# aleximmer/Laplace

Hardware: AMD Instinct MI355X
Metric: KFAC-GGN fit samples/sec, ResNet-18 (higher is better)
Workload: dtype f32 (fp16x2-split products, fp32 accumulate); 1 GPU; c4: ResNet-18 (CIFAR stem, BN frozen) full-network KFAC exact GGN fit, per-GPU minibatch 128, synthetic N(0,1) 3x32x32, 10 classes, N=50000; per_gpu_batch=128, parallelism=dp1, minibatches_in_flight=2

## Files before the change

### include/laplace_hip.h

```cpp
#ifndef LAPLACE_HIP_H
#define LAPLACE_HIP_H

#include <stddef.h>
#include <stdint.h>

#ifdef __cplusplus
extern "C" {
#endif

#define LK_OK 0
#define LK_EINVAL (-1)
#define LK_EWORKSPACE (-2)
#define LK_ELAUNCH (-3)
#define LK_ENOTCONV (-4)

#define LK_GRAM_UPPER_ONLY 1u
#define LK_GRAM_SLABS_PERSIST 2u

int lk_version(void);
const char* lk_last_error(void);

size_t lk_loss_workspace_bytes(int64_t B);
int lk_softmax_hess_sqrt_f32(const float* f, const int64_t* y, int64_t B, int64_t C, float* S,
                             float* loss_accum, float* ws, void* stream);
// ... 125 lines not shown
int lk_copy_absmax_f32(const float* x, float* y, int64_t n, unsigned* amax, void* stream);

int lk_pack_upper_f32(const float* A, int64_t n, float* packed, void* stream);
int lk_unpack_upper_f32(const float* packed, int64_t n, float* A, void* stream);

int lk_gemm_f32(const float* A, const float* B, const float* E, float* C, int64_t batch, int64_t M, int64_t N, int64_t K,
                int64_t lda, int64_t ldb, int64_t ldc, int64_t lde, int64_t stride_a, int64_t stride_b, int64_t stride_c,
                int trans_a, int trans_b, float alpha, int accumulate, void* stream);
int lk_kron_pow_f32(const float* l1, int64_t n1, const float* l2, int64_t n2, const float* delta, float exponent,
                    int damping, float* lam, void* stream);
int lk_unsplit_transpose_f32(const void* x_h, const void* x_l, const int* sexp, int64_t S, int64_t B, int64_t L, int64_t C,
                             float* out, void* stream);
size_t lk_gram_tn_f16x2_workspace_bytes(int64_t R, int64_t C);
int lk_gram_tn_f16x2(const void* x_h, const void* x_l, const int* sexp, int64_t R, int64_t C, float alpha, float* G,
                     const void* zero16, void* ws, size_t ws_bytes, void* stream);

int lk_diag_ggn_linear_f32(const float* a, const float* g, int64_t B, int64_t Cc, int64_t Di, int64_t Do,
                           float alpha, float* h_w, float* h_b, void* stream);

int lk_jac_linear_f32(const float* a, const float* g, int64_t B, int64_t Cc, int64_t Di, int64_t Do,
                      float* Js, int64_t P, int64_t col0, int64_t bcol0, void* stream);
int lk_jac_conv_f32(const float* x_nchw, const float* g, int64_t B, int64_t Cc, int64_t Cin, int64_t H, int64_t W,
                    int64_t Do, int kh, int kw, int sh, int sw, int ph, int pw, int dh, int dw,
                    float* Js, int64_t P, int64_t col0, int64_t bcol0, void* stream);

int lk_jac_norm_affine_f32(const float* g, const float* xhat, int64_t S, int64_t B, int64_t L, int64_t Ch, int layout,
                           float* Js, int64_t P, int64_t wcol0, int64_t bcol0, void* stream);

int lk_jac_norm_affine_nhwc_f16x2(const void* g_h, const void* g_l, const int* sexp, const float* x, const float* mu,
                                  const float* rstd, int64_t S, int64_t B, int64_t L, int64_t Ch, float* Js, int64_t P,
// ... 157 lines not shown
```

### laplace_amd/_lib.py

```python
from __future__ import annotations

import ctypes
import os
from typing import Optional

import torch

_HERE = os.path.dirname(os.path.abspath(__file__))
LIB_PATH = os.environ.get("LK_LIB") or os.path.join(_HERE, "csrc", "liblaplace_hip.so")

LK_GRAM_UPPER_ONLY = 1
LK_GRAM_SLABS_PERSIST = 2

_c_f32p = ctypes.c_void_p
_i64 = ctypes.c_int64
_int = ctypes.c_int
_f32 = ctypes.c_float
_sz = ctypes.c_size_t
_vp = ctypes.c_void_p
_u32 = ctypes.c_uint

SIGNATURES = {
    "lk_version": (_int, []),
    "lk_last_error": (ctypes.c_char_p, []),
# ... 43 lines not shown
    "lk_conv_nhwc_f16x2_vjp": (_int, [_vp, _vp, _vp, _vp, _i64, _i64, _i64, _i64, _vp, _vp, _vp, _vp, _i64, _i64, _i64, _i64,
                                      _vp, _vp, _vp, _vp, _vp, _vp, _int, _vp, _i64, _vp, _vp, _vp, _vp, _vp,
                                      _vp, _int, _vp]),
    "lk_conv_winp_eligible": (_int, [_i64, _i64, _i64, _i64, _i64, _i64, _int]),
    "lk_conv_nhwc_f16x2_vjp_wc": (_int, [_vp, _vp, _vp, _vp, _i64, _i64, _i64, _i64, _vp, _vp, _vp, _vp, _vp, _vp, _i64, _i64, _i64,
                                         _i64, _vp, _vp, _vp, _vp, _vp, _vp, _int, _vp, _i64, _vp, _vp, _vp, _vp, _vp, _vp, _int,
                                         _vp]),
    "lk_conv_nhwc_f16x2_vjp_strided": (_int, [_vp] * 16 + [_i64] * 9 + [_vp, _vp, _vp, _vp, _vp, _vp, _int, _vp, _i64, _vp, _vp, _vp,
                                               _vp, _vp, _vp, _int, _vp]),
    "lk_vjp_nhwc_split_f16x2": (_int, [_vp, _vp, _vp, _vp, _vp, _vp, _int, _vp, _vp, _vp, _i64, _i64, _i64, _vp, _vp, _vp, _vp]),
    "lk_bn_act_fwd_nhwc_f16x2": (_int, [_vp, _vp, _i64, _vp, _vp, _vp, _vp, _vp, _vp, _vp, _vp, _i64, _int, _i64, _i64, _i64, _vp, _vp,
                                        _vp, _vp, _vp, _vp, _vp, _vp]),
    "lk_unsplit_transpose_f32": (_int, [_vp, _vp, _vp, _i64, _i64, _i64, _i64, _vp, _vp]),
    "lk_gram_tn_f16x2_workspace_bytes": (_sz, [_i64, _i64]),
    "lk_gram_tn_f16x2": (_int, [_vp, _vp, _vp, _i64, _i64, _f32, _vp, _vp, _vp, _sz, _vp]),
    "lk_gemm_f32": (_int, [_vp, _vp, _vp, _vp, _i64, _i64, _i64, _i64, _i64, _i64, _i64, _i64, _i64, _i64, _i64, _int, _int, _f32,
                           _int, _vp]),
    "lk_kron_pow_f32": (_int, [_vp, _i64, _vp, _i64, _vp, _f32, _int, _vp, _vp]),
    "lk_pack_upper_f32": (_int, [_vp, _i64, _vp, _vp]),
    "lk_unpack_upper_f32": (_int, [_vp, _i64, _vp, _vp]),
    "lk_symmetrize_f32": (_int, [_vp, _i64, _vp]),
    "lk_permute_sym_f32": (_int, [_vp, _i64, _i64, _vp, _int, _vp]),
    "lk_finalize_factors_f32": (_int, [_i64, _vp, _vp, _vp, _vp, _vp, _vp, _vp]),
    "lk_diag_ggn_linear_f32": (_int, [_vp, _vp, _i64, _i64, _i64, _i64, _f32, _vp, _vp, _vp]),
    "lk_jac_linear_f32": (_int, [_vp, _vp, _i64, _i64, _i64, _i64, _vp, _i64, _i64, _i64, _vp]),
    "lk_jac_conv_f32": (
        _int,
        [_vp, _vp, _i64, _i64, _i64, _i64, _i64, _i64, _int, _int, _int, _int, _int, _int, _int, _int, _vp, _i64, _i64, _i64, _vp],
    ),
    "lk_jac_gconv_f32": (
# ... 700 lines not shown
    def gram_tn_f16x2(self, x, alpha, out):
        _check(out, "out")
        _one_scale(x, "gram_tn_f16x2")
        C = x.planes.shape[-1]
        R = x.planes[0].numel() // C
        nbytes = int(self.lib.lk_gram_tn_f16x2_workspace_bytes(R, C))
        if nbytes == 0 and R:
            raise LaplaceHipError(f"gram_tn_f16x2: C = {C} not supported (64 or a multiple of 128)")
        ws = self._workspace(nbytes, out.device)
        z = self._zero16(out.device)
        self._rc(self._timed("gram16", float(R) * C * (C + 1), out.device, lambda: self.lib.lk_gram_tn_f16x2(
            _ptr(x.planes[0]), _ptr(x.planes[1]), _ptr(x.sexp), R, C, float(alpha), _ptr(out), _ptr(z), _ptr(ws),
            ws.numel(), self._stream(out.device))), "lk_gram_tn_f16x2")
        return out

    def pack_upper(self, A, packed):
        _check(A, "A"), _check(packed, "packed")
        self._rc(self.lib.lk_pack_upper_f32(_ptr(A), A.shape[0], _ptr(packed), self._stream(A.device)), "lk_pack_upper_f32")

    def unpack_upper(self, packed, A):
        _check(A, "A"), _check(packed, "packed")
        self._rc(self.lib.lk_unpack_upper_f32(_ptr(packed), A.shape[0], _ptr(A), self._stream(A.device)), "lk_unpack_upper_f32")

    def gemm(self, A, B, C, batch, M, N, Kd, lda, ldb, ldc, sa=0, sb=0, sc=0, ta=False, tb=False, E=None, lde=0,
             alpha=1.0, accumulate=False):
        self._rc(self.lib.lk_gemm_f32(_ptr(A), _ptr(B), _ptr(E), _ptr(C), batch, M, N, Kd, lda, ldb, ldc, lde, sa, sb, sc,
                                      1 if ta else 0, 1 if tb else 0, float(alpha), 1 if accumulate else 0,
                                      self._stream(C.device)), "lk_gemm_f32")

    def kron_pow(self, l1, l2, delta, exponent, damping=False):
# ... 1002 lines not shown
```

### laplace_amd/backend.py

```python
from __future__ import annotations

import collections
import math
import threading
import os
from collections.abc import MutableMapping

import torch
import torch.nn.functional as F
from torch import nn

from laplace_amd._lib import SplitTensor, get_kernels, is_channels_last, keep_layout
from laplace_amd.capture import NormTapReused, Tape, norm_servable
from laplace_amd.sweep import SeedBatchedSweep, SweepUnsupported
from laplace_amd.sweep_nhwc import NhwcNormGrad, SplitSweep
from laplace_amd.kron import HipKron
from laplace_amd.refapi import EFInterface, GGNInterface


_OWN_ROTATION = True


def shared_operands(tap, g, B, C, Q1=None, Q2=None, bounds=None, planes: bool = True):
    m = tap.module
# ... 357 lines not shown
    def _positions(tap, a) -> int:
        if tap.kind == "conv2d":
            m = tap.module
            H, W = a.shape[-2:]
            oh = (H + 2 * m.padding[0] - m.dilation[0] * (m.kernel_size[0] - 1) - 1) // m.stride[0] + 1
            ow = (W + 2 * m.padding[1] - m.dilation[1] * (m.kernel_size[1] - 1) - 1) // m.stride[1] + 1
            return oh * ow
        return int(a[0].numel() // a.shape[-1])

    def _factor_shapes(self, tap):
        m = tap.module
        if tap.kind == "linear":
            return m.out_features, m.in_features
        return m.out_channels, m.in_channels * m.kernel_size[0] * m.kernel_size[1]

    def _factor_A(self, tap, N, alpha_a_scale, kfac_approx, A, fused=False):
        K = get_kernels()
        a = tap.a.to(torch.float32)
        m = tap.module
        L = self._positions(tap, a)
        if tap.kind == "linear":
            Di = m.in_features
            if kfac_approx == "expand" or L == 1:
                K.gram_tn(a.reshape(-1, Di).contiguous(), alpha_a_scale / (N * L), A, upper_only=fused)
            else:
                K.gram_tn(a.reshape(a.shape[0], L, Di).mean(1).contiguous(), alpha_a_scale / N, A, upper_only=fused)
            return A
        if kfac_approx == "expand":
            ak = keep_layout(a)
            n = A.shape[0]
            if (fused and getattr(K, "use_gram_conv16", False) and hasattr(K, "im2col_split") and m.kernel_size[0] * m.kernel_size[1] > 1
                    and tuple(m.dilation) == (1, 1) and m.stride[0] == m.stride[1] and m.padding[0] == m.padding[1]
                    and m.groups == 1 and isinstance(m.padding[0], int) and ak.is_cuda == A.is_cuda
                    and (n + 127) // 128 * 128 <= 4096 and ak.shape[0] * L * ((n + 127) // 128 * 128) < (1 << 33)):
                Kp = n if (n == 64 or n % 128 == 0) else (64 if n < 64 else (n + 127) // 128 * 128)
                pm = K.im2col_split(ak, m.kernel_size, m.stride[0], m.padding[0], Kp)
                if Kp == n:
                    K.gram_tn_f16x2(pm, alpha_a_scale / (N * L), A)
                else:
                    Ap = torch.zeros(Kp, Kp, dtype=torch.float32, device=A.device)
                    K.gram_tn_f16x2(pm, alpha_a_scale / (N * L), Ap)
                    A += Ap[:n, :n]
                return A
            K.gram_conv(ak, m.kernel_size, m.stride, m.padding, m.dilation, alpha_a_scale / (N * L), A,
                        upper_only=fused, native=fused)
        else:
            cols = torch.nn.functional.unfold(a, m.kernel_size, dilation=m.dilation, padding=m.padding, stride=m.stride)
            if fused:
                KK = m.kernel_size[0] * m.kernel_size[1]
                cols = cols.reshape(cols.shape[0], m.in_channels, KK, -1).transpose(1, 2).reshape(cols.shape)
            K.gram_tn(cols.mean(2).contiguous(), alpha_a_scale / N, A, upper_only=fused)
        return A
# ... 265 lines not shown
_PROCESS_STREAMS_LOCK = threading.Lock()


def _process_streams(key, make):
    with _PROCESS_STREAMS_LOCK:
        return _process_streams_locked(key, make)


def _process_streams_locked(key, make):
    hit = _PROCESS_STREAMS.get(key)
    if hit is None:
        hit = _PROCESS_STREAMS[key] = make()
    return hit


class KronAccumulator:

    use_pixgram = True
    _defer_bn = True
    _persist_slabs = True
    pix_group = 8
    lag_join = True

    def __init__(self, backend, N: int, kfac_approx: str = "expand", overlap: bool = True):
        twin, dt = backend._twin() if hasattr(backend, "_twin") else (None, torch.float32)
        self._caller, self._out_dtype = (backend, dt) if twin is not None else (None, torch.float32)
        if twin is not None:
            backend = twin
        self.backend, self.N, self.kfac_approx = backend, N, kfac_approx
        self.overlap = overlap
# ... 72 lines not shown
            plan = K.pixpair_plan(H, W, Cin, tap.a.device)
            if plan is not None and plan[0] * Cin * Cin * 4 <= (1 << 30):
                return ("pair", H, W, Cin, plan)
        if H * W <= K.pixgram_max_hw and H * W * Cin <= 16384:
            return ("dense", H, W, Cin)
        return None

    def _accumulate_A(self, idx, tap, F, rt):
        K = get_kernels()
        if self.defer_pix:
            geo = self._pix_geometry(tap)
            if geo is not None and geo[0] == "pair" and tap.a.dtype == torch.float32:
                t = K.nchw_to_nhwc(keep_layout(tap.a))
                self._pix_inputs.setdefault(idx, []).append((geo, rt / (self.N * geo[1] * geo[2]), t, tap.module))
                return
            self.backend._factor_A(tap, self.N, rt, self.kfac_approx, F[1], fused=True)
            return
        acc = self._pix.get(idx)
        if acc is None:
            self.backend._factor_A(tap, self.N, rt, self.kfac_approx, F[1], fused=True)
            return
        geo, buf = acc
        alpha = rt / (self.N * geo[1] * geo[2])
        a = keep_layout(tap.a.to(torch.float32))
        if geo[0] != "pair":
            K.pixgram_accumulate(a, alpha, buf)
        elif self.pix_group <= 1:
            K.pixpair_accumulate(a, alpha, buf, geo[4])
        else:
            self._push_pix_input(idx, geo, alpha, a, nhwc=False)

    direct_stack = True

    def _pix_sink(self, name, shape, device):
        idx = self._tap_index.get(name)
# ... 430 lines not shown
            main = torch.cuda.current_stream(f.device)
            side.wait_stream(main)
            with torch.cuda.stream(side):
                for i, (tap, F) in enumerate(zip(tape.taps, self.factors)):
                    self._accumulate_A(i, tap, F, rt)
            self._a_done = torch.cuda.Event()
            self._a_done.record(side)
        else:
            for i, (tap, F) in enumerate(zip(tape.taps, self.factors)):
                self._accumulate_A(i, tap, F, rt)
        seeds, hs = b._kron_seeds(f, y, self.loss)
        defer = getattr(grad_fn, "streams_taps", False) and self._defer_bn
        if getattr(grad_fn, "streams_taps", False):
            by_name = {tap.name: (tap, F) for tap, F in zip(tape.taps, self.factors)}

            def on_tap(name, g):
                tap, F = by_name[name]
                persist = None if isinstance(g, SplitTensor) else self._g_slabs(tap, g, rt * hs)
                if side is None:
                    b._factor_G(tap, g, rt * hs, self.kfac_approx, F[0], fused=True, persist=persist)
                    return
                ev = torch.cuda.Event()
                ev.record(main)
                side.wait_event(ev)
                with torch.cuda.stream(side):
                    b._factor_G(tap, g, rt * hs, self.kfac_approx, F[0], fused=True, persist=persist)
                (g.planes if isinstance(g, SplitTensor) else g).record_stream(side)
                if isinstance(g, SplitTensor) and torch.is_tensor(g.sexp):
                    g.sexp.record_stream(side)

            grad_fn(seeds, stack=False, on_tap=on_tap, defer_bn_scale=defer)
        else:
            grads = grad_fn(seeds, stack=False)
            for tap, g, F in zip(tape.taps, grads, self.factors):
                b._factor_G(tap, g, rt * hs, self.kfac_approx, F[0], fused=True)
        if defer:
            self._note_grad_scales(tape, grad_fn.grad_scale())
        if side is not None:
            if self.lag_join:
                for tap in tape.taps:
                    if torch.is_tensor(tap.a) and tap.a.is_cuda:
                        tap.a.record_stream(side)
                if self._side_done is not None:
                    self._side_older.append(self._side_done)
                while len(self._side_older) >= self.lag_depth and self._side_older:
                    main.wait_event(self._side_older.pop(0))
# ... 8 lines not shown
            return None
        K = get_kernels()
        S, B, Do = g.shape[0], g.shape[1], g.shape[2]
        L = g.shape[3] * g.shape[4]
        need = K.gram_nt_slab_bytes(S * B, Do, L)
        idx = self._tap_index[tap.name]
        cur = self._gslabs.get(idx)
        if cur is not None and (cur[0].numel() < need or cur[2] != L or cur[3] != alpha):
            self._flush_g_slabs(only=idx)
            cur = None
        if cur is None:
            cur = (torch.zeros(need, dtype=torch.uint8, device=g.device), Do, L, alpha)
            self._gslabs[idx] = cur
        return cur[0]

    def _raw_tensors(self):
        return [t for F in self.factors for t in F] + [self.loss]

    def _raw_compatible(self, other) -> bool:
        return (self.factors is not None and other.factors is not None and not other._pix
                and not other._pix_pending and not self._gslabs and not other._gslabs
                and (not (self._pix or self._pix_pending) or all(g[0] == "pair" for g, _ in self._pix.values()))
                and self.N == other.N and self.kfac_approx == other.kfac_approx and self.backend is other.backend
                and self._taps_meta == other._taps_meta and len(self.factors) == len(other.factors)
                and all(a.shape == b.shape for a, b in zip(self._raw_tensors(), other._raw_tensors()))
                and set(self._gscale) == set(other._gscale)
                and all(self._gscale[k] is other._gscale[k] or torch.equal(self._gscale[k], other._gscale[k])
                        for k in self._gscale))

    def clone(self) -> "KronAccumulator":
        self._fold_lanes()
        self._join_side()
        new = KronAccumulator(self.backend, self.N, self.kfac_approx, self.overlap)
        new._caller, new._out_dtype, new.coalesce = self._caller, self._out_dtype, self.coalesce
        new.use_pixgram, new._persist_slabs = self.use_pixgram, self._persist_slabs
        new.defer_pix, new.pix_group = self.defer_pix, self.pix_group
        new._pix_inputs = {k: list(v) for k, v in self._pix_inputs.items()}
        if self.factors is not None:
            if self._gslabs or any(g[0] != "pair" for g, _ in self._pix.values()):
                raise RuntimeError("clone() of an accumulator with dense pixel-pair / slab state is not supported")
            for idx in list(self._pix_pending):
                self._drain_pixpair(idx)
            new.factors = [[t.clone() for t in F] for F in self.factors]
            new.loss = self.loss.clone()
            new._taps_meta = list(self._taps_meta)
            new._gscale = dict(self._gscale)
            new._tap_index = dict(self._tap_index)
            new._pix = {idx: (geo, buf.clone()) for idx, (geo, buf) in self._pix.items()}
            new._pix_pending, new._gslabs = {}, {}
            new._side = self._side
        return new

    def merge_(self, other: "KronAccumulator") -> bool:
        self._fold_lanes()
        other._fold_lanes()
        if not self._raw_compatible(other):
            return False
        skip = set(other._pix_inputs)
        mine = [t for i, F in enumerate(self.factors) for j, t in enumerate(F) if not (j == 1 and i in skip)] + [self.loss]
        theirs = [t for i, F in enumerate(other.factors) for j, t in enumerate(F) if not (j == 1 and i in skip)] + [other.loss]
        side = self._side or other._side
        if side is None or not self.lag_join or not self.loss.is_cuda:
            self._join_side()
            other._join_side()
            torch._foreach_add_(mine, theirs)
            self._push_adopted(self._adopt_pix_inputs(other))
        else:
            self._side = side
            main = torch.cuda.current_stream(self.loss.device)
            if self._side_done is not None:
# ... 11 lines not shown
            self._side_done = torch.cuda.Event()
            self._side_done.record(side)
        return True

    def _join_side(self):
        if self._side is not None:
            torch.cuda.current_stream(self._side.device).wait_stream(self._side)
            self._side_done = None
            self._side_older = []

    def _flush_g_slabs(self, only=None):
        K = get_kernels()
        if self._gslabs:
            self._join_side()
        for idx in ([only] if only is not None else list(self._gslabs)):
            buf, n, L, alpha = self._gslabs.pop(idx)
            K.gram_slabs_reduce(buf, n, L, alpha, self.factors[idx][0], upper_only=True)

    def _note_grad_scales(self, tape, scales):
        for idx, tap in enumerate(tape.taps):
            s_new = scales.get(tap.name)
            s_old = self._gscale.get(idx)
            if s_old is None:
                if s_new is not None:
                    self._gscale[idx] = s_new
            elif s_new is None or (s_new is not s_old and not torch.equal(s_new, s_old)):
                raise RuntimeError(f"{tap.name}: the BatchNorm scale changed during the fit (model not in eval mode?)")

    def _apply_grad_scales(self):
        self._join_side()
        for idx, s_ in self._gscale.items():
            G = self.factors[idx][0]
            G.mul_(s_.reshape(-1, 1) * s_.reshape(1, -1))
        self._gscale = {}

    def tensors(self) -> list[torch.Tensor]:
        self._fold_lanes()
        self._resolve_pix_inputs()
        self._flush_pixgrams()
        self._flush_g_slabs()
        self._apply_grad_scales()
        out = CurvatureExchange([t for F in self.factors for t in F] + [self.loss])
        out.owner = self
        return out

    def finalize(self):
        K = get_kernels()
        rt = math.sqrt(float(self.backend.factor))
# ... 212 lines not shown
```

### laplace_amd/csrc/lk_sweep16.hip

```cpp
#include "lk_common.h"
#include "lk_split16.h"

namespace lk {

typedef short s16x4 __attribute__((ext_vector_type(4)));

template <bool MFLOAT>
__global__ __launch_bounds__(256) void vjp_nhwc_split_kernel(
    const float* __restrict__ g, const unsigned* __restrict__ g_amax, const _Float16* __restrict__ g2h,
    const _Float16* __restrict__ g2l, const int* __restrict__ g2_sexp, const void* __restrict__ m,
    const unsigned* __restrict__ m_amax, const float* __restrict__ scale, const unsigned* __restrict__ scale_amax, int C,
    int S, int64_t per8, _Float16* __restrict__ oh, _Float16* __restrict__ ol, int* __restrict__ out_sexp) {
  float bound = 0.f;
  if (g) bound += __uint_as_float(g_amax[0]);
  const VjpScale vs = vjp_bound_scale<true>(bound, g2h != nullptr, g2_sexp, m != nullptr, MFLOAT, m_amax, scale != nullptr, scale_amax);
  const float sc_out = exp2i_sat(vs.so);
  if (blockIdx.x == 0 && threadIdx.x == 0) out_sexp[0] = vs.so;
  const int64_t e8 = (int64_t)blockIdx.x * 256 + threadIdx.x;
  if (e8 >= per8) return;
  float mult[8];
#pragma unroll
  for (int j = 0; j < 8; ++j) mult[j] = sc_out;
  if (m) {
    if (MFLOAT) vjp_mult8_times(mult, reinterpret_cast<const float*>(m) + 8 * e8);
// ... 136 lines not shown
__device__ __forceinline__ float gram16_unscale_add(float old, float v, float alpha, float inv) {
  return __builtin_fmaf(alpha, (v * inv) * inv, old);
}

typedef __attribute__((address_space(3))) void lds_void16;
typedef __attribute__((address_space(1))) const void gbl_void16;

struct Gram16Tnp {
  const int* tiles;
  int ldc;
  const int* sexp;
  float alpha;
  float* blocks;
};

template <int NB, int BKR, int KW, bool TNP>
__global__ __launch_bounds__(256) void gram16_kernel(const _Float16* __restrict__ Xh, const _Float16* __restrict__ Xl,
                                                     int64_t R, int64_t C, int64_t rows_per_split,
                                                     const _Float16* __restrict__ zero16, float* __restrict__ ws,
                                                     int nbc, const Gram16Tnp tp) {
  using G = Gram16Cfg<NB, BKR, KW>;
  constexpr int TW = G::TW;
  extern __shared__ __attribute__((aligned(16))) char smem[];
  const int tid = threadIdx.x, lane = tid & 63, wave = tid >> 6;
  int bi = 0, bj = 0;
  int64_t colA = 0, colB = 0, out_off = 0;
  if constexpr (TNP) {
    const int nblk = gridDim.x;
    int bid = blockIdx.x;
    bid = xcd_tile_order(bid, nblk);
    colA = tp.tiles[3 * bid], colB = tp.tiles[3 * bid + 1], out_off = tp.tiles[3 * bid + 2];
  } else {
    int p = blockIdx.x;
    while (p >= nbc - bi) p -= nbc - bi, ++bi;
    bj = bi + p;
    colA = (int64_t)bi * NB, colB = (int64_t)bj * NB;
  }
// ... 45 lines not shown

  auto load_frag = [&](const char* plane, int k16, int col0) -> f16x8 {
    s16x4 v[2];
#pragma unroll
    for (int j = 0; j < 2; ++j) {
      const int row = k16 * 16 + f_row + j * 4;
      const int col = col0 + f_col;
      const int off = row * G::PITCH + (((col >> 5) ^ gram16_swz<NB>(row)) << 6) + (col & 31) * 2;
      const unsigned addr = (unsigned)(uintptr_t)(__attribute__((address_space(3))) const char*)(plane + off);
      asm volatile("ds_read_b64_tr_b16 %0, %1" : "=v"(v[j]) : "v"(addr));
    }
    const f16x4 f0 = __builtin_bit_cast(f16x4, v[0]), f1 = __builtin_bit_cast(f16x4, v[1]);
    return f16x8{f0[0], f0[1], f0[2], f0[3], f1[0], f1[1], f1[2], f1[3]};
  };

  constexpr int NOLD = TNP ? (KW == 4 ? TW * TW * 4 : TW * TW * 16) : 1;
  float old[NOLD];
  if constexpr (TNP) {
    const int lr_ = lane & 31, lh_ = lane >> 5;
    if (KW == 4) {
#pragma unroll
      for (int i = 0; i < NOLD; ++i) {
        const int e = tid + 256 * i, t = e >> 10, a = t / TW, b = t % TW, row = (e >> 5) & 31, col = e & 31;
        old[i] = tp.blocks[out_off + (int64_t)(a * 32 + row) * tp.ldc + b * 32 + col];
      }
    } else {
#pragma unroll
      for (int a = 0; a < TW; ++a)
#pragma unroll
        for (int b = 0; b < TW; ++b)
#pragma unroll
          for (int r = 0; r < 16; ++r) {
// ... 33 lines not shown
#pragma unroll
      for (int a = 0; a < TW; ++a)
#pragma unroll
        for (int b = 0; b < TW; ++b) {
          if (diag && wr == wc && a > b) continue;
          f32x16 c = acc[a][b];
          c = __builtin_amdgcn_mfma_f32_32x32x16_f16(al[a], bh[b], c, 0, 0, 0);
          c = __builtin_amdgcn_mfma_f32_32x32x16_f16(ah[a], bl[b], c, 0, 0, 0);
          c = __builtin_amdgcn_mfma_f32_32x32x16_f16(ah[a], bh[b], c, 0, 0, 0);
          acc[a][b] = c;
        }
    }
  }

  const int lr = lane & 31, lh = lane >> 5;
  float* blk = TNP ? nullptr : ws + ((int64_t)blockIdx.y * gridDim.x + blockIdx.x) * (NB * NB);
  if (KW == 4) {
    __syncthreads();
    float* red = reinterpret_cast<float*>(smem);
#pragma unroll
    for (int a = 0; a < TW; ++a)
#pragma unroll
      for (int b = 0; b < TW; ++b) {
        if (!TNP && a > b) continue;
#pragma unroll
        for (int r = 0; r < 16; ++r) {
          const int row = (r & 3) + 8 * (r >> 2) + 4 * lh;
          red[((wave * TW + a) * TW + b) * 1024 + row * 32 + lr] = acc[a][b][r];
        }
      }
    __syncthreads();
    float inv = 0.f;
    if constexpr (TNP) inv = exp2i_sat(-tp.sexp[0]);
#pragma unroll
    for (int i = 0; i < TW * TW * 4; ++i) {
      const int e = tid + 256 * i;
      const int t = e >> 10, a = t / TW, b = t % TW;
      if (!TNP && a > b) continue;
      const float v = ((red[e] + red[TW * TW * 1024 + e]) + red[2 * TW * TW * 1024 + e]) + red[3 * TW * TW * 1024 + e];
      const int row = (e >> 5) & 31, col = e & 31;
      if constexpr (TNP) tp.blocks[out_off + (int64_t)(a * 32 + row) * tp.ldc + b * 32 + col] = gram16_unscale_add(old[i], v, tp.alpha, inv);
      else blk[(a * 32 + row) * NB + b * 32 + col] = v;
    }
    return;
  }
  if (!wave_active) return;
  float inv = 0.f;
  if constexpr (TNP) inv = exp2i_sat(-tp.sexp[0]);
#pragma unroll
  for (int a = 0; a < TW; ++a)
#pragma unroll
    for (int b = 0; b < TW; ++b) {
      if (diag && wr == wc && a > b) continue;
#pragma unroll
      for (int r = 0; r < 16; ++r) {
        const int row = wr * 64 + a * 32 + (r & 3) + 8 * (r >> 2) + 4 * lh;
        const int col = wc * 64 + b * 32 + lr;
        if constexpr (TNP)
          tp.blocks[out_off + (int64_t)row * tp.ldc + col] = gram16_unscale_add(old[(a * TW + b) * 16 + r], acc[a][b][r], tp.alpha, inv);
        else blk[row * NB + col] = acc[a][b][r];
      }
    }
}

template <int NB>
__global__ __launch_bounds__(256) void gram16_reduce4_kernel(const float* __restrict__ ws, int nparts, int npairs, int nbc,
                                                             int C, const int* __restrict__ sexp, float alpha,
                                                             float* __restrict__ Gm) {
  __shared__ float4 red[4][64];
  const int pair = blockIdx.y;
  int bi = 0, bj = 0;
  {
    int p = pair;
    while (p >= nbc - bi) p -= nbc - bi, ++bi;
// ... 91 lines not shown
             "lk_unsplit_transpose_f32: bad arguments (S * B <= 65535)");
  LK_REQUIRE(L <= 65535 * 32ll, "lk_unsplit_transpose_f32: L too large for grid.y (L <= %lld positions)", 65535 * 32ll);
  LK_REQUIRE(C < (1ll << 31) - 32, "lk_unsplit_transpose_f32: C too large (C < 2^31 - 32 channels)");
  if (S * B == 0 || L == 0 || C == 0) return LK_OK;
  hipLaunchKernelGGL(unsplit_transpose_kernel, dim3((unsigned)((C + 31) / 32), (unsigned)((L + 31) / 32), (unsigned)(S * B)),
                     dim3(256), 0, (hipStream_t)stream, (const _Float16*)x_h, (const _Float16*)x_l, sexp, (int)S, (int)B,
                     (int)L, (int)C, out);
  return check_launch("unsplit_transpose_kernel");
}

namespace {
struct Gram16Plan {
  int nb, nbc, npairs, kw, bkr;
  int64_t nsplit, rows_per_split, nparts;
};
Gram16Plan gram16_plan(int64_t R, int64_t C) {
  Gram16Plan p;
  p.nb = C == 64 ? 64 : 128;
  p.kw = C == 64 ? 4 : 1;
  p.bkr = C == 64 ? 64 : 32;
  p.nbc = (int)(C / p.nb);
  p.npairs = p.nbc * (p.nbc + 1) / 2;
  int64_t want = (512 + p.npairs - 1) / p.npairs;
  int64_t stages = (R + p.bkr - 1) / p.bkr;
  int64_t per = (stages + want - 1) / want;
  if (per < 8) per = 8;
  p.rows_per_split = per * p.bkr;
  p.nsplit = (R + p.rows_per_split - 1) / p.rows_per_split;
  if (p.nsplit < 1) p.nsplit = 1;
  p.nparts = p.nsplit;
  return p;
}
}

extern "C" size_t lk_gram_tn_f16x2_workspace_bytes(int64_t R, int64_t C) {
  if (C < 64 || (C != 64 && C % 128)) return 0;
  const Gram16Plan p = gram16_plan(R, C);
  return (size_t)p.nparts * p.npairs * p.nb * p.nb * sizeof(float);
}

extern "C" int lk_gram_tn_f16x2(const void* x_h, const void* x_l, const int* sexp, int64_t R, int64_t C, float alpha,
                                float* Gm, const void* zero16, void* ws, size_t ws_bytes, void* stream) {
  LK_REQUIRE(x_h && x_l && sexp && Gm && zero16 && ws && R >= 0, "lk_gram_tn_f16x2: null pointer");
  LK_REQUIRE(C == 64 || (C >= 128 && C % 128 == 0 && C <= 4096), "lk_gram_tn_f16x2: C must be 64 or a multiple of 128");
  if (R == 0) return LK_OK;
  const Gram16Plan p = gram16_plan(R, C);
  LK_REQUIRE(ws_bytes >= lk_gram_tn_f16x2_workspace_bytes(R, C), "lk_gram_tn_f16x2: workspace too small");
  hipStream_t st = (hipStream_t)stream;
  dim3 grid((unsigned)p.npairs, (unsigned)p.nsplit);
  if (C == 64) {
    using Gc = Gram16Cfg<64, 64, 4>;
    hipLaunchKernelGGL((gram16_kernel<64, 64, 4, false>), grid, dim3(256), 2 * Gc::STAGE, st, (const _Float16*)x_h,
                       (const _Float16*)x_l, R, C, p.rows_per_split, (const _Float16*)zero16, (float*)ws, p.nbc, Gram16Tnp{});
  } else {
    using Gc = Gram16Cfg<128, 32, 1>;
    hipLaunchKernelGGL((gram16_kernel<128, 32, 1, false>), grid, dim3(256), 2 * Gc::STAGE, st, (const _Float16*)x_h,
                       (const _Float16*)x_l, R, C, p.rows_per_split, (const _Float16*)zero16, (float*)ws, p.nbc, Gram16Tnp{});
  }
  int rc = check_launch("gram16_kernel");
  if (rc != LK_OK) return rc;
  dim3 rgrid((unsigned)(p.nb * p.nb / 256), (unsigned)p.npairs);
  if (C == 64)
    hipLaunchKernelGGL(gram16_reduce4_kernel<64>, rgrid, dim3(256), 0, st, (const float*)ws, (int)p.nparts, p.npairs, p.nbc,
                       (int)C, sexp, alpha, Gm);
  else
    hipLaunchKernelGGL(gram16_reduce4_kernel<128>, rgrid, dim3(256), 0, st, (const float*)ws, (int)p.nparts, p.npairs, p.nbc,
                       (int)C, sexp, alpha, Gm);
  return check_launch("gram16_reduce4_kernel");
}

namespace lk {
struct Pix13Args {
  const _Float16 *xh, *xl;
  const _Float16* zero16;
  const int* slots;
  const int* sexp;
  float* blocks;
  float alpha;
  int R, H, W;
};

__device__ __forceinline__ f16x8 pix13_frag(unsigned plane, int lane, int col0) {
  const int grp = lane >> 4, r16 = lane & 15;
// ... 145 lines not shown
extern "C" int lk_conv3x3_pixpair_accumulate_f16x2(const void* x_h, const void* x_l, const int* sexp, int64_t B, int64_t H,
                                                   int64_t W, int64_t Cin, float alpha, float* blocks,
                                                   const int32_t* tiles_dev, int64_t n_tiles, const void* zero16,
                                                   void* stream) {
  LK_REQUIRE(x_h && x_l && sexp && blocks && tiles_dev && zero16 && B >= 0 && n_tiles >= 0,
             "lk_conv3x3_pixpair_accumulate_f16x2: bad arguments");
  LK_REQUIRE(Cin >= 64 && Cin % 64 == 0 && n_tiles < (1ll << 31) && H * W * Cin < (1ll << 31),
             "lk_conv3x3_pixpair_accumulate_f16x2: needs Cin % 64 == 0");
  if (B == 0 || n_tiles == 0) return LK_OK;
  Gram16Tnp tp;
  tp.tiles = tiles_dev, tp.ldc = (int)Cin, tp.sexp = sexp, tp.alpha = alpha, tp.blocks = blocks;
  hipStream_t st = (hipStream_t)stream;
  const int64_t ld = H * W * Cin;
  if (Cin % 128) {
    using Gc = Gram16Cfg<64, 64, 4>;
    hipLaunchKernelGGL((gram16_kernel<64, 64, 4, true>), dim3((unsigned)n_tiles), dim3(256), 2 * Gc::STAGE, st,
                       (const _Float16*)x_h, (const _Float16*)x_l, B, ld, B, (const _Float16*)zero16, (float*)nullptr, 0, tp);
  } else {
    using Gc = Gram16Cfg<128, 32, 1>;
    hipLaunchKernelGGL((gram16_kernel<128, 32, 1, true>), dim3((unsigned)n_tiles), dim3(256), 2 * Gc::STAGE, st,
                       (const _Float16*)x_h, (const _Float16*)x_l, B, ld, B, (const _Float16*)zero16, (float*)nullptr, 0, tp);
  }
  return check_launch("gram16_kernel<pixel pairs>");
}
```

Baseline: 21190 samples/s.

## Accumulate f16x2 Gram factors into persistent slabs and batch same-shape layers per launch

Adds a persistent-slab mode for the fp16x2 Gram kernel: each minibatch's contribution is read-modify-written into per-layer slab buffers, and the cross-split reduction into the Kronecker factor is deferred to flush time instead of running every minibatch. Gradient taps of identical shape are grouped (up to 8) into a single launch using a z-dimension layer table, and the split plan accounts for the layer count. This is meant to cut per-minibatch reduce kernels and launch overhead, at the cost of extra slab memory and a read of the old slab values in every accumulate.

Measured after the change: 21290 samples/s (median of 6 runs). Within noise of the previous version (+0.5%).

```diff
diff --git a/include/laplace_hip.h b/include/laplace_hip.h
--- a/include/laplace_hip.h
+++ b/include/laplace_hip.h
@@ -163,6 +163,13 @@
 size_t lk_gram_tn_f16x2_workspace_bytes(int64_t R, int64_t C);
 int lk_gram_tn_f16x2(const void* x_h, const void* x_l, const int* sexp, int64_t R, int64_t C, float alpha, float* G,
                      const void* zero16, void* ws, size_t ws_bytes, void* stream);
+int lk_gram16_plan(int64_t R, int64_t C, int layers, int64_t* out);
+size_t lk_gram16_slab_bytes(int64_t R, int64_t C, int layers);
+int lk_gram16_accumulate(const void* const* x_h, const void* const* x_l, const int* const* sexp, const float* alpha,
+                         float* const* slabs, int layers, int64_t R, int64_t C, size_t slab_bytes, const void* zero16,
+                         void* stream);
+int lk_gram16_slabs_reduce(const float* slabs, size_t slab_bytes, int64_t R, int64_t C, int layers, float* G,
+                           const void* zero16, void* stream);
 
 int lk_diag_ggn_linear_f32(const float* a, const float* g, int64_t B, int64_t Cc, int64_t Di, int64_t Do,
                            float alpha, float* h_w, float* h_b, void* stream);
diff --git a/laplace_amd/_lib.py b/laplace_amd/_lib.py
--- a/laplace_amd/_lib.py
+++ b/laplace_amd/_lib.py
@@ -81,6 +81,10 @@
     "lk_unsplit_transpose_f32": (_int, [_vp, _vp, _vp, _i64, _i64, _i64, _i64, _vp, _vp]),
     "lk_gram_tn_f16x2_workspace_bytes": (_sz, [_i64, _i64]),
     "lk_gram_tn_f16x2": (_int, [_vp, _vp, _vp, _i64, _i64, _f32, _vp, _vp, _vp, _sz, _vp]),
+    "lk_gram16_plan": (_int, [_i64, _i64, _int, _vp]),
+    "lk_gram16_slab_bytes": (_sz, [_i64, _i64, _int]),
+    "lk_gram16_accumulate": (_int, [_vp, _vp, _vp, _vp, _vp, _int, _i64, _i64, _sz, _vp, _vp]),
+    "lk_gram16_slabs_reduce": (_int, [_vp, _sz, _i64, _i64, _int, _vp, _vp, _vp]),
     "lk_gemm_f32": (_int, [_vp, _vp, _vp, _vp, _i64, _i64, _i64, _i64, _i64, _i64, _i64, _i64, _i64, _i64, _i64, _int, _int, _f32,
                            _int, _vp]),
     "lk_kron_pow_f32": (_int, [_vp, _i64, _vp, _i64, _vp, _f32, _int, _vp, _vp]),
@@ -811,6 +815,50 @@
             ws.numel(), self._stream(out.device))), "lk_gram_tn_f16x2")
         return out
 
+    use_gram16_persist = True
+    gram16_group = True
+    GRAM16_MAX_LAYERS = 8
+
+    def gram16_plan(self, R, C, layers=1):
+        o = (ctypes.c_int64 * 4)()
+        if self.lib.lk_gram16_plan(int(R), int(C), int(layers), o) != 0:
+            return None
+        return dict(nb=o[0], npairs=o[1], nsplit=o[2], rows_per_split=o[3])
+
+    def gram16_slab_bytes(self, R, C, layers=1) -> int:
+        return int(self.lib.lk_gram16_slab_bytes(int(R), int(C), int(layers)))
+
+    def gram16_accumulate(self, xs, alphas, slabs):
+        n = len(xs)
+        if not 1 <= n <= self.GRAM16_MAX_LAYERS or len(alphas) != n or len(slabs) != n:
+            raise LaplaceHipError(f"gram16_accumulate: 1 to {self.GRAM16_MAX_LAYERS} layers, one alpha and one slab buffer each")
+        C = xs[0].planes.shape[-1]
+        R = xs[0].planes[0].numel() // C
+        for x, s in zip(xs, slabs):
+            _one_scale(x, "gram16_accumulate")
+            _check(s, "slabs")
+            if x.planes.shape[-1] != C or x.planes[0].numel() != R * C:
+                raise LaplaceHipError("gram16_accumulate: the layers of one launch share [rows, C]")
+        nbytes = self.gram16_slab_bytes(R, C, n)
+        if nbytes == 0 and R:
+            raise LaplaceHipError(f"gram16_accumulate: C = {C} not supported (64 or a multiple of 128)")
+        if min(s.numel() for s in slabs) * 4 < nbytes:
+            raise LaplaceHipError("gram16_accumulate: persistent slab buffer too small")
+        dev = slabs[0].device
+        arr = lambda ts: (ctypes.c_void_p * n)(*[t.data_ptr() for t in ts])
+        xh, xl, se, sl = arr([x.planes[0] for x in xs]), arr([x.planes[1] for x in xs]), arr([x.sexp for x in xs]), arr(slabs)
+        al = (ctypes.c_float * n)(*[float(a) for a in alphas])
+        z = self._zero16(dev)
+        self._rc(self._timed("gram16", float(n) * R * C * (C + 1), dev, lambda: self.lib.lk_gram16_accumulate(
+            xh, xl, se, al, sl, n, R, C, nbytes, _ptr(z), self._stream(dev))), "lk_gram16_accumulate")
+
+    def gram16_slabs_reduce(self, slabs, R, C, layers, out):
+        _check(out, "out"), _check(slabs, "slabs")
+        self._rc(self.lib.lk_gram16_slabs_reduce(_ptr(slabs), slabs.numel() * 4, int(R), int(C), int(layers), _ptr(out),
+                                                 _ptr(self._zero16(out.device)), self._stream(out.device)),
+                 "lk_gram16_slabs_reduce")
+        return out
+
     def pack_upper(self, A, packed):
         _check(A, "A"), _check(packed, "packed")
         self._rc(self.lib.lk_pack_upper_f32(_ptr(A), A.shape[0], _ptr(packed), self._stream(A.device)), "lk_pack_upper_f32")
diff --git a/laplace_amd/backend.py b/laplace_amd/backend.py
--- a/laplace_amd/backend.py
+++ b/laplace_amd/backend.py
@@ -395,7 +395,7 @@
             return m.out_features, m.in_features
         return m.out_channels, m.in_channels * m.kernel_size[0] * m.kernel_size[1]
 
-    def _factor_A(self, tap, N, alpha_a_scale, kfac_approx, A, fused=False):
+    def _factor_A(self, tap, N, alpha_a_scale, kfac_approx, A, fused=False, slabs16=None):
         K = get_kernels()
         a = tap.a.to(torch.float32)
         m = tap.module
@@ -416,7 +416,9 @@
                     and (n + 127) // 128 * 128 <= 4096 and ak.shape[0] * L * ((n + 127) // 128 * 128) < (1 << 33)):
                 Kp = n if (n == 64 or n % 128 == 0) else (64 if n < 64 else (n + 127) // 128 * 128)
                 pm = K.im2col_split(ak, m.kernel_size, m.stride[0], m.padding[0], Kp)
-                if Kp == n:
+                if slabs16 is not None:
+                    K.gram16_accumulate([pm], [alpha_a_scale / (N * L)], [slabs16(pm, Kp, n)])
+                elif Kp == n:
                     K.gram_tn_f16x2(pm, alpha_a_scale / (N * L), A)
                 else:
                     Ap = torch.zeros(Kp, Kp, dtype=torch.float32, device=A.device)
@@ -712,6 +714,29 @@
     return hit
 
 
+class Gram16Groups:
+
+    def __init__(self, group_max):
+        self.group_max = max(int(group_max), 1)
+        self.held = []
+
+    def _take(self):
+        group, self.held = self.held, []
+        return group
+
+    def add(self, idx, g):
+        out = []
+        if self.held and (tuple(self.held[0][1].shape) != tuple(g.shape) or any(i == idx for i, _ in self.held)):
+            out.append(self._take())
+        self.held.append((idx, g))
+        if g.shape[-1] < 128 or len(self.held) >= self.group_max:
+            out.append(self._take())
+        return out
+
+    def end(self):
+        return [self._take()] if self.held else []
+
+
 class KronAccumulator:
 
     use_pixgram = True
@@ -814,11 +839,11 @@
                 t = K.nchw_to_nhwc(keep_layout(tap.a))
                 self._pix_inputs.setdefault(idx, []).append((geo, rt / (self.N * geo[1] * geo[2]), t, tap.module))
                 return
-            self.backend._factor_A(tap, self.N, rt, self.kfac_approx, F[1], fused=True)
+            self.backend._factor_A(tap, self.N, rt, self.kfac_approx, F[1], fused=True, slabs16=self._a16_slabs(idx))
             return
         acc = self._pix.get(idx)
         if acc is None:
-            self.backend._factor_A(tap, self.N, rt, self.kfac_approx, F[1], fused=True)
+            self.backend._factor_A(tap, self.N, rt, self.kfac_approx, F[1], fused=True, slabs16=self._a16_slabs(idx))
             return
         geo, buf = acc
         alpha = rt / (self.N * geo[1] * geo[2])
@@ -1279,8 +1304,37 @@
         if getattr(grad_fn, "streams_taps", False):
             by_name = {tap.name: (tap, F) for tap, F in zip(tape.taps, self.factors)}
 
+            K16 = get_kernels()
+            persist16 = bool(getattr(K16, "use_gram16_persist", False)) and self._persist_slabs and self.kfac_approx == "expand"
+            group_max = int(getattr(K16, "GRAM16_MAX_LAYERS", 1)) if persist16 and getattr(K16, "gram16_group", False) else 1
+            groups = Gram16Groups(group_max)
+
+            def launch(group):
+                idxs, gs = [i for i, _ in group], [g for _, g in group]
+                C = gs[0].shape[-1]
+                R = gs[0].planes[0].numel() // C
+                slabs = [self._g16_slabs(("g16", i), R, C, len(gs), gs[0].planes.device) for i in idxs]
+                if side is None:
+                    K16.gram16_accumulate(gs, [rt * hs] * len(gs), slabs)
+                    return
+                ev = torch.cuda.Event()
+                ev.record(main)
+                side.wait_event(ev)
+                with torch.cuda.stream(side):
+                    K16.gram16_accumulate(gs, [rt * hs] * len(gs), slabs)
+                for g in gs:
+                    g.planes.record_stream(side)
+                    g.sexp.record_stream(side)
+
             def on_tap(name, g):
                 tap, F = by_name[name]
+                if persist16 and isinstance(g, SplitTensor) and torch.is_tensor(g.sexp) and g.sexp.numel() == 1 \
+                        and (g.shape[-1] == 64 or g.shape[-1] % 128 == 0) and g.shape[-1] <= 4096:
+                    for group in groups.add(self._tap_index[name], g):
+                        launch(group)
+                    return
+                for group in groups.end():
+                    launch(group)
                 persist = None if isinstance(g, SplitTensor) else self._g_slabs(tap, g, rt * hs)
                 if side is None:
                     b._factor_G(tap, g, rt * hs, self.kfac_approx, F[0], fused=True, persist=persist)
@@ -1294,7 +1348,12 @@
                 if isinstance(g, SplitTensor) and torch.is_tensor(g.sexp):
                     g.sexp.record_stream(side)
 
-            grad_fn(seeds, stack=False, on_tap=on_tap, defer_bn_scale=defer)
+            try:
+                grad_fn(seeds, stack=False, on_tap=on_tap, defer_bn_scale=defer)
+                for group in groups.end():
+                    launch(group)
+            finally:
+                groups.held = []
         else:
             grads = grad_fn(seeds, stack=False)
             for tap, g, F in zip(tape.taps, grads, self.factors):
@@ -1333,6 +1392,22 @@
             self._gslabs[idx] = cur
         return cur[0]
 
+    def _g16_slabs(self, key, R, C, layers, device, n=None):
+        cur = self._gslabs.get(key)
+        if cur is not None and cur[1:4] != (R, C, layers):
+            self._flush_g_slabs(only=key)
+            cur = None
+        if cur is None:
+            nbytes = get_kernels().gram16_slab_bytes(R, C, layers)
+            cur = (torch.zeros(nbytes // 4, dtype=torch.float32, device=device), R, C, layers, n)
+            self._gslabs[key] = cur
+        return cur[0]
+
+    def _a16_slabs(self, idx):
+        if not (self._persist_slabs and getattr(get_kernels(), "use_gram16_persist", False)):
+            return None
+        return lambda pm, Kp, n: self._g16_slabs(("a16", idx), pm.planes[0].numel() // Kp, Kp, 1, pm.planes.device, n)
+
     def _raw_tensors(self):
         return [t for F in self.factors for t in F] + [self.loss]
 
@@ -1356,6 +1431,7 @@
         new.defer_pix, new.pix_group = self.defer_pix, self.pix_group
         new._pix_inputs = {k: list(v) for k, v in self._pix_inputs.items()}
         if self.factors is not None:
+            self._flush_g_slabs()
             if self._gslabs or any(g[0] != "pair" for g, _ in self._pix.values()):
                 raise RuntimeError("clone() of an accumulator with dense pixel-pair / slab state is not supported")
             for idx in list(self._pix_pending):
@@ -1373,6 +1449,9 @@
     def merge_(self, other: "KronAccumulator") -> bool:
         self._fold_lanes()
         other._fold_lanes()
+        for acc in (self, other):
+            if acc.factors is not None:
+                acc._flush_g_slabs()
         if not self._raw_compatible(other):
             return False
         skip = set(other._pix_inputs)
@@ -1414,6 +1493,18 @@
         if self._gslabs:
             self._join_side()
         for idx in ([only] if only is not None else list(self._gslabs)):
+            if isinstance(idx, tuple):
+                buf, R, C, layers, n = self._gslabs.pop(idx)
+                F = self.factors[idx[1]][0 if idx[0] == "g16" else 1]
+                if n is None or n == C:
+                    K.gram16_slabs_reduce(buf, R, C, layers, F)
+                else:
+                    Fp = torch.zeros(C, C, dtype=torch.float32, device=F.device)
+                    K.gram16_slabs_reduce(buf, R, C, layers, Fp)
+                    F += Fp[:n, :n]
+                if buf.is_cuda:
+                    buf.record_stream(torch.cuda.current_stream(buf.device))
+                continue
             buf, n, L, alpha = self._gslabs.pop(idx)
             K.gram_slabs_reduce(buf, n, L, alpha, self.factors[idx][0], upper_only=True)
 
@@ -1432,6 +1523,8 @@
         for idx, s_ in self._gscale.items():
             G = self.factors[idx][0]
             G.mul_(s_.reshape(-1, 1) * s_.reshape(1, -1))
+        if self._gscale:
+            self._defer_bn = False
         self._gscale = {}
 
     def tensors(self) -> list[torch.Tensor]:
diff --git a/laplace_amd/csrc/lk_sweep16.hip b/laplace_amd/csrc/lk_sweep16.hip
--- a/laplace_amd/csrc/lk_sweep16.hip
+++ b/laplace_amd/csrc/lk_sweep16.hip
@@ -174,13 +174,32 @@
   float* blocks;
 };
 
-template <int NB, int BKR, int KW, bool TNP>
+constexpr int GRAM16_MAX_LAYERS = 8;
+struct Gram16Layer {
+  const _Float16 *xh, *xl;
+  const int* sexp;
+  float* slabs;
+  float alpha;
+};
+struct Gram16Batch {
+  Gram16Layer l[GRAM16_MAX_LAYERS];
+};
+
+template <int NB, int BKR, int KW, bool ACC, bool TNP>
 __global__ __launch_bounds__(256) void gram16_kernel(const _Float16* __restrict__ Xh, const _Float16* __restrict__ Xl,
                                                      int64_t R, int64_t C, int64_t rows_per_split,
                                                      const _Float16* __restrict__ zero16, float* __restrict__ ws,
-                                                     int nbc, const Gram16Tnp tp) {
+                                                     int nbc, const Gram16Tnp tp, const Gram16Batch bt) {
   using G = Gram16Cfg<NB, BKR, KW>;
   constexpr int TW = G::TW;
+  static_assert(!(ACC && TNP), "the pixel-pair form owns its blocks already");
+  constexpr bool RMW = ACC || TNP;
+  float acc_alpha = 0.f;
+  const int* acc_sexp = nullptr;
+  if constexpr (ACC) {
+    const Gram16Layer& ly = bt.l[blockIdx.z];
+    Xh = ly.xh, Xl = ly.xl, ws = ly.slabs, acc_alpha = ly.alpha, acc_sexp = ly.sexp;
+  }
   extern __shared__ __attribute__((aligned(16))) char smem[];
   const int tid = threadIdx.x, lane = tid & 63, wave = tid >> 6;
   int bi = 0, bj = 0;
@@ -256,8 +275,30 @@
     return f16x8{f0[0], f0[1], f0[2], f0[3], f1[0], f1[1], f1[2], f1[3]};
   };
 
-  constexpr int NOLD = TNP ? (KW == 4 ? TW * TW * 4 : TW * TW * 16) : 1;
+  constexpr int NOLD = RMW ? (KW == 4 ? TW * TW * 4 : TW * TW * 16) : 1;
   float old[NOLD];
+  [[maybe_unused]] float* const acc_blk = ACC ? ws + ((int64_t)blockIdx.y * gridDim.x + blockIdx.x) * (NB * NB) : nullptr;
+  if constexpr (ACC) {
+    const int lr_ = lane & 31, lh_ = lane >> 5;
+    if (KW == 4) {
+#pragma unroll
+      for (int i = 0; i < NOLD; ++i) {
+        const int e = tid + 256 * i, t = e >> 10, a = t / TW, b = t % TW, row = (e >> 5) & 31, col = e & 31;
+        old[i] = a > b ? 0.f : acc_blk[(a * 32 + row) * NB + b * 32 + col];
+      }
+    } else if (wave_active) {
+#pragma unroll
+      for (int a = 0; a < TW; ++a)
+#pragma unroll
+        for (int b = 0; b < TW; ++b)
+#pragma unroll
+          for (int r = 0; r < 16; ++r) {
+            const int row = wr * 64 + a * 32 + (r & 3) + 8 * (r >> 2) + 4 * lh_;
+            const int col = wc * 64 + b * 32 + lr_;
+            old[(a * TW + b) * 16 + r] = (diag && wr == wc && a > b) ? 0.f : acc_blk[row * NB + col];
+          }
+    }
+  }
   if constexpr (TNP) {
     const int lr_ = lane & 31, lh_ = lane >> 5;
     if (KW == 4) {
@@ -321,7 +362,7 @@
   }
 
   const int lr = lane & 31, lh = lane >> 5;
-  float* blk = TNP ? nullptr : ws + ((int64_t)blockIdx.y * gridDim.x + blockIdx.x) * (NB * NB);
+  float* blk = RMW ? nullptr : ws + ((int64_t)blockIdx.y * gridDim.x + blockIdx.x) * (NB * NB);
   if (KW == 4) {
     __syncthreads();
     float* red = reinterpret_cast<float*>(smem);
@@ -339,6 +380,7 @@
     __syncthreads();
     float inv = 0.f;
     if constexpr (TNP) inv = exp2i_sat(-tp.sexp[0]);
+    if constexpr (ACC) inv = exp2i_sat(-acc_sexp[0]);
 #pragma unroll
     for (int i = 0; i < TW * TW * 4; ++i) {
       const int e = tid + 256 * i;
@@ -347,6 +389,7 @@
       const float v = ((red[e] + red[TW * TW * 1024 + e]) + red[2 * TW * TW * 1024 + e]) + red[3 * TW * TW * 1024 + e];
       const int row = (e >> 5) & 31, col = e & 31;
       if constexpr (TNP) tp.blocks[out_off + (int64_t)(a * 32 + row) * tp.ldc + b * 32 + col] = gram16_unscale_add(old[i], v, tp.alpha, inv);
+      else if constexpr (ACC) acc_blk[(a * 32 + row) * NB + b * 32 + col] = gram16_unscale_add(old[i], v, acc_alpha, inv);
       else blk[(a * 32 + row) * NB + b * 32 + col] = v;
     }
     return;
@@ -354,6 +397,7 @@
   if (!wave_active) return;
   float inv = 0.f;
   if constexpr (TNP) inv = exp2i_sat(-tp.sexp[0]);
+  if constexpr (ACC) inv = exp2i_sat(-acc_sexp[0]);
 #pragma unroll
   for (int a = 0; a < TW; ++a)
 #pragma unroll
@@ -365,6 +409,8 @@
         const int col = wc * 64 + b * 32 + lr;
         if constexpr (TNP)
           tp.blocks[out_off + (int64_t)row * tp.ldc + col] = gram16_unscale_add(old[(a * TW + b) * 16 + r], acc[a][b][r], tp.alpha, inv);
+        else if constexpr (ACC)
+          acc_blk[row * NB + col] = gram16_unscale_add(old[(a * TW + b) * 16 + r], acc[a][b][r], acc_alpha, inv);
         else blk[row * NB + col] = acc[a][b][r];
       }
     }
@@ -486,14 +532,15 @@
   int nb, nbc, npairs, kw, bkr;
   int64_t nsplit, rows_per_split, nparts;
 };
-Gram16Plan gram16_plan(int64_t R, int64_t C) {
+Gram16Plan gram16_plan(int64_t R, int64_t C, int layers = 1) {
   Gram16Plan p;
   p.nb = C == 64 ? 64 : 128;
   p.kw = C == 64 ? 4 : 1;
   p.bkr = C == 64 ? 64 : 32;
   p.nbc = (int)(C / p.nb);
   p.npairs = p.nbc * (p.nbc + 1) / 2;
-  int64_t want = (512 + p.npairs - 1) / p.npairs;
+  const int64_t tiles = (int64_t)p.npairs * layers;
+  int64_t want = (512 + tiles - 1) / tiles;
   int64_t stages = (R + p.bkr - 1) / p.bkr;
   int64_t per = (stages + want - 1) / want;
   if (per < 8) per = 8;
@@ -522,12 +569,12 @@
   dim3 grid((unsigned)p.npairs, (unsigned)p.nsplit);
   if (C == 64) {
     using Gc = Gram16Cfg<64, 64, 4>;
-    hipLaunchKernelGGL((gram16_kernel<64, 64, 4, false>), grid, dim3(256), 2 * Gc::STAGE, st, (const _Float16*)x_h,
-                       (const _Float16*)x_l, R, C, p.rows_per_split, (const _Float16*)zero16, (float*)ws, p.nbc, Gram16Tnp{});
+    hipLaunchKernelGGL((gram16_kernel<64, 64, 4, false, false>), grid, dim3(256), 2 * Gc::STAGE, st, (const _Float16*)x_h,
+                       (const _Float16*)x_l, R, C, p.rows_per_split, (const _Float16*)zero16, (float*)ws, p.nbc, Gram16Tnp{}, Gram16Batch{});
   } else {
     using Gc = Gram16Cfg<128, 32, 1>;
-    hipLaunchKernelGGL((gram16_kernel<128, 32, 1, false>), grid, dim3(256), 2 * Gc::STAGE, st, (const _Float16*)x_h,
-                       (const _Float16*)x_l, R, C, p.rows_per_split, (const _Float16*)zero16, (float*)ws, p.nbc, Gram16Tnp{});
+    hipLaunchKernelGGL((gram16_kernel<128, 32, 1, false, false>), grid, dim3(256), 2 * Gc::STAGE, st, (const _Float16*)x_h,
+                       (const _Float16*)x_l, R, C, p.rows_per_split, (const _Float16*)zero16, (float*)ws, p.nbc, Gram16Tnp{}, Gram16Batch{});
   }
   int rc = check_launch("gram16_kernel");
   if (rc != LK_OK) return rc;
@@ -539,6 +586,109 @@
     hipLaunchKernelGGL(gram16_reduce4_kernel<128>, rgrid, dim3(256), 0, st, (const float*)ws, (int)p.nparts, p.npairs, p.nbc,
                        (int)C, sexp, alpha, Gm);
   return check_launch("gram16_reduce4_kernel");
+}
+
+static int gram16_check_shape(const char* fn, int64_t R, int64_t C, int layers) {
+  LK_REQUIRE(layers >= 1 && layers <= GRAM16_MAX_LAYERS, "%s: layers out of range (1 <= layers <= %d)", fn, GRAM16_MAX_LAYERS);
+  LK_REQUIRE(C == 64 || (C >= 128 && C % 128 == 0 && C <= 4096), "%s: C must be 64 or a multiple of 128 (<= 4096)", fn);
+  LK_REQUIRE(R >= 0 && R < (1ll << 40) / C, "%s: extent out of range (0 <= R, R * C < 2^40)", fn);
+  return LK_OK;
+}
+
+static bool gram16_shape_ok(int64_t R, int64_t C, int layers) {
+  return layers >= 1 && layers <= GRAM16_MAX_LAYERS && (C == 64 || (C >= 128 && C % 128 == 0 && C <= 4096)) && R >= 0 &&
+         R < (1ll << 40) / C;
+}
+
+static int gram16_check_plan(int64_t R, int64_t C, int layers, const int64_t* out) {
+  LK_REQUIRE(out, "lk_gram16_plan: null pointer");
+  return gram16_check_shape("lk_gram16_plan", R, C, layers);
+}
+
+static size_t gram16_slab_bytes(int64_t R, int64_t C, int layers) {
+  const Gram16Plan p = gram16_plan(R, C, layers);
+  return (size_t)p.nsplit * p.npairs * p.nb * p.nb * sizeof(float);
+}
+
+static int gram16_check_accumulate(const void* const* x_h, const void* const* x_l, const int* const* sexp, const float* alpha,
+                                   float* const* slabs, int layers, int64_t R, int64_t C, size_t slab_bytes,
+                                   const void* zero16) {
+  const char* fn = "lk_gram16_accumulate";
+  LK_REQUIRE(x_h && x_l && sexp && alpha && slabs && zero16, "%s: null pointer", fn);
+  int rc = gram16_check_shape(fn, R, C, layers);
+  if (rc != LK_OK) return rc;
+  for (int i = 0; i < layers; ++i)
+    LK_REQUIRE(x_h[i] && x_l[i] && sexp[i] && slabs[i], "%s: null pointer in the table entry of layer %d", fn, i);
+  for (int i = 0; i < layers; ++i)
+    for (int j = i + 1; j < layers; ++j)
+      LK_REQUIRE(slabs[i] != slabs[j], "%s: layers %d and %d share their slabs (a tile has one writer per launch)", fn, i, j);
+  LK_REQUIRE(slab_bytes >= gram16_slab_bytes(R, C, layers), "%s: slabs too small (lk_gram16_slab_bytes, each layer's own)", fn);
+  return LK_OK;
+}
+
+static int gram16_check_reduce(const float* slabs, size_t slab_bytes, int64_t R, int64_t C, int layers, const float* Gm,
+                               const void* zero16) {
+  const char* fn = "lk_gram16_slabs_reduce";
+  LK_REQUIRE(slabs && Gm && zero16, "%s: null pointer", fn);
+  int rc = gram16_check_shape(fn, R, C, layers);
+  if (rc != LK_OK) return rc;
+  LK_REQUIRE(slab_bytes >= gram16_slab_bytes(R, C, layers), "%s: slabs too small (lk_gram16_slab_bytes)", fn);
+  return LK_OK;
+}
+
+extern "C" int lk_gram16_plan(int64_t R, int64_t C, int layers, int64_t* out) {
+  int rc = gram16_check_plan(R, C, layers, out);
+  if (rc != LK_OK) return rc;
+  const Gram16Plan p = gram16_plan(R, C, layers);
+  out[0] = p.nb, out[1] = p.npairs, out[2] = p.nsplit, out[3] = p.rows_per_split;
+  return LK_OK;
+}
+
+extern "C" size_t lk_gram16_slab_bytes(int64_t R, int64_t C, int layers) {
+  return gram16_shape_ok(R, C, layers) ? gram16_slab_bytes(R, C, layers) : 0;
+}
+
+extern "C" int lk_gram16_accumulate(const void* const* x_h, const void* const* x_l, const int* const* sexp,
+                                    const float* alpha, float* const* slabs, int layers, int64_t R, int64_t C,
+                                    size_t slab_bytes, const void* zero16, void* stream) {
+  int rc = gram16_check_accumulate(x_h, x_l, sexp, alpha, slabs, layers, R, C, slab_bytes, zero16);
+  if (rc != LK_OK || R == 0) return rc;
+  Gram16Batch bt{};
+  for (int i = 0; i < layers; ++i) {
+    bt.l[i].xh = (const _Float16*)x_h[i], bt.l[i].xl = (const _Float16*)x_l[i], bt.l[i].sexp = sexp[i];
+    bt.l[i].slabs = slabs[i], bt.l[i].alpha = alpha[i];
+  }
+  const Gram16Plan p = gram16_plan(R, C, layers);
+  dim3 grid((unsigned)p.npairs, (unsigned)p.nsplit, (unsigned)layers);
+  hipStream_t st = (hipStream_t)stream;
+  if (C == 64) {
+    using Gc = Gram16Cfg<64, 64, 4>;
+    hipLaunchKernelGGL((gram16_kernel<64, 64, 4, true, false>), grid, dim3(256), 2 * Gc::STAGE, st, (const _Float16*)nullptr,
+                       (const _Float16*)nullptr, R, C, p.rows_per_split, (const _Float16*)zero16, (float*)nullptr, p.nbc,
+                       Gram16Tnp{}, bt);
+  } else {
+    using Gc = Gram16Cfg<128, 32, 1>;
+    hipLaunchKernelGGL((gram16_kernel<128, 32, 1, true, false>), grid, dim3(256), 2 * Gc::STAGE, st, (const _Float16*)nullptr,
+                       (const _Float16*)nullptr, R, C, p.rows_per_split, (const _Float16*)zero16, (float*)nullptr, p.nbc,
+                       Gram16Tnp{}, bt);
+  }
+  return check_launch("gram16_kernel<persistent slabs>");
+}
+
+extern "C" int lk_gram16_slabs_reduce(const float* slabs, size_t slab_bytes, int64_t R, int64_t C, int layers, float* Gm,
+                                      const void* zero16, void* stream) {
+  int rc = gram16_check_reduce(slabs, slab_bytes, R, C, layers, Gm, zero16);
+  if (rc != LK_OK || R == 0) return rc;
+  const Gram16Plan p = gram16_plan(R, C, layers);
+  dim3 rgrid((unsigned)(p.nb * p.nb / 256), (unsigned)p.npairs);
+  hipStream_t st = (hipStream_t)stream;
+  if (C == 64)
+    hipLaunchKernelGGL(gram16_reduce4_kernel<64>, rgrid, dim3(256), 0, st, slabs, (int)p.nparts, p.npairs, p.nbc, (int)C,
+                       (const int*)zero16, 1.f, Gm);
+  else
+    hipLaunchKernelGGL(gram16_reduce4_kernel<128>, rgrid, dim3(256), 0, st, slabs, (int)p.nparts, p.npairs, p.nbc, (int)C,
+                       (const int*)zero16, 1.f, Gm);
+  return check_launch("gram16_reduce4_kernel<persistent slabs>");
 }
 
 namespace lk {
@@ -714,12 +864,14 @@
   const int64_t ld = H * W * Cin;
   if (Cin % 128) {
     using Gc = Gram16Cfg<64, 64, 4>;
-    hipLaunchKernelGGL((gram16_kernel<64, 64, 4, true>), dim3((unsigned)n_tiles), dim3(256), 2 * Gc::STAGE, st,
-                       (const _Float16*)x_h, (const _Float16*)x_l, B, ld, B, (const _Float16*)zero16, (float*)nullptr, 0, tp);
+    hipLaunchKernelGGL((gram16_kernel<64, 64, 4, false, true>), dim3((unsigned)n_tiles), dim3(256), 2 * Gc::STAGE, st,
+                       (const _Float16*)x_h, (const _Float16*)x_l, B, ld, B, (const _Float16*)zero16, (float*)nullptr, 0, tp,
+                       Gram16Batch{});
   } else {
     using Gc = Gram16Cfg<128, 32, 1>;
-    hipLaunchKernelGGL((gram16_kernel<128, 32, 1, true>), dim3((unsigned)n_tiles), dim3(256), 2 * Gc::STAGE, st,
-                       (const _Float16*)x_h, (const _Float16*)x_l, B, ld, B, (const _Float16*)zero16, (float*)nullptr, 0, tp);
+    hipLaunchKernelGGL((gram16_kernel<128, 32, 1, false, true>), dim3((unsigned)n_tiles), dim3(256), 2 * Gc::STAGE, st,
+                       (const _Float16*)x_h, (const _Float16*)x_l, B, ld, B, (const _Float16*)zero16, (float*)nullptr, 0, tp,
+                       Gram16Batch{});
   }
   return check_launch("gram16_kernel<pixel pairs>");
 }
```
